# utiasSTARS/GraphIK

Hardware: AMD Instinct MI355X
Metric: IK solves/sec (batched random goals) (higher is better)
Workload: dtype f64

## Files before the change

graphik_amd/csrc/gik_rtr.hip.h:

```cpp
#pragma once

#include <hip/hip_runtime.h>

#include <type_traits>

#include "gik_wave.hip.h"

namespace gik {

#define UNI(cond) (__builtin_amdgcn_ballot_w64(cond) != 0ull)

__device__ inline bool plain_in_exec(double mv, double mp, double dHd, double e, double T, double beta, double rr,
                                     double t2hi, int j, int jmax_v) {
  unsigned long long ok, saved;
  asm volatile("s_mov_b64 %1, exec\n\t"
               "v_cmpx_lt_f64_e64 %0, %2, %3\n\t"
               "v_cmpx_gt_f64_e64 %0, %4, 0\n\t"
               "v_cmpx_gt_i32_e64 %0, %11, %10\n\t"
               "v_cmpx_lt_f64_e64 %0, %5, %6\n\t"
               "v_cmpx_ge_f64_e64 %0, %7, %8\n\t"
               "v_cmpx_nle_f64_e64 %0, %9, %12\n\t"
               "s_mov_b64 exec, %1"
               : "=&s"(ok), "=&s"(saved)
               : "s"(mv), "v"(mp), "s"(dHd), "v"(e), "v"(T), "v"(beta), "s"(1e-3), "v"(rr), "s"(j), "v"(jmax_v),
                 "v"(t2hi));
  return ok != 0ull;
}

struct RtrOut {
  double f, gradnorm;
  int iterations, inner_total, stop, n_accept;
  int inner_executed;
  double Delta;
  int paused;
};

struct RtrResume {
  double Delta;
  int kiter, inner_total, inner_exec, n_accept;
  int resumed;
  int resumes;
};

template <typename Ctx>
__device__ inline double grad_norm_and_rho(Ctx &cx, double g, double (&rho0)[Ctx::NC]) {
  if constexpr (Ctx::NC == 3) {
    double v[4] = {g * g, g * cx.Q[0], g * cx.Q[1], g * cx.Q[2]};
    cx.template sum_n<4>(v);
#pragma unroll
    for (int m = 0; m < 3; ++m) rho0[m] = v[m + 1];
    return sqrt(v[0]);
  }
  double v[Ctx::NC + 1];
  v[0] = g * g;
#pragma unroll
  for (int m = 0; m < Ctx::NC; ++m) v[m + 1] = g * cx.pk2[m];
  cx.template sum_n<Ctx::NC + 1>(v);
#pragma unroll
  for (int m = 0; m < Ctx::NC; ++m) rho0[m] = v[m + 1];
  return sqrt(v[0]);
}

__device__ inline double boundary_tau(double e_Pd2, double d_Pd, double Delta2, double e_Pe) {
  const double e_Pd = 0.5 * e_Pd2;
  return (sqrt(fma(e_Pd, e_Pd, d_Pd * (Delta2 - e_Pe))) - e_Pd) / d_Pd;
}

struct MigCtl {
  int *credits;
  int *simd_run;
  int sid;
  const unsigned int *fresh;
  const int *y_avail;
  const unsigned int *y_tail;
  int B;
  unsigned int y_cap;
  const unsigned int *done;
  int waves;
  int slice_cycles;
};
enum { PAUSE_NONE = 0, PAUSE_DONATE = 1, PAUSE_YIELD = 2 };

template <typename Ctx>
__device__ inline bool mig_poll(const Ctx &cx, const MigCtl &m) {
  int go = 0;
  if (cx.lead()) {
    if (__hip_atomic_load(m.credits, __ATOMIC_RELAXED, __HIP_MEMORY_SCOPE_AGENT) > 0 &&
        __hip_atomic_load(&m.simd_run[m.sid], __ATOMIC_RELAXED, __HIP_MEMORY_SCOPE_AGENT) >= 2) {
      if (__hip_atomic_fetch_add(m.credits, -1, __ATOMIC_RELAXED, __HIP_MEMORY_SCOPE_AGENT) >= 1)
        go = 1;
      else
        __hip_atomic_fetch_add(m.credits, 1, __ATOMIC_RELAXED, __HIP_MEMORY_SCOPE_AGENT);
    }
  }
  return __builtin_amdgcn_readfirstlane(go) != 0;
}

template <typename Ctx>
__device__ inline bool mig_anyone_waiting(const Ctx &cx, const MigCtl &m) {
  int w = 0;
  if (cx.lead()) {
    const unsigned int yt = __hip_atomic_load(m.y_tail, __ATOMIC_RELAXED, __HIP_MEMORY_SCOPE_AGENT);
    const unsigned int dn = __hip_atomic_load(m.done, __ATOMIC_RELAXED, __HIP_MEMORY_SCOPE_AGENT);
    w = yt + (unsigned)m.waves + 64u < m.y_cap && (unsigned)m.B > dn + (unsigned)m.waves;
  }
  return __builtin_amdgcn_readfirstlane(w) != 0;
}

template <typename Ctx, typename = void>
struct split_ehess : std::false_type {};
template <typename Ctx>
struct split_ehess<Ctx, std::enable_if_t<Ctx::SPLIT_EHESS>> : std::true_type {};

template <int K, bool THETA_ONE, bool SLICE, typename Ctx, bool MIG = false>
__device__ inline void rtr_solve_one(Ctx &cx, const Params &p, const gik_trace &trace, int has_trace,
                                     int dbg, double *dbg_buf, int b, double &x, RtrOut &out,
                                     const RtrResume &rs, int slice_its, const MigCtl *mig = nullptr) {
  static_assert(!MIG || SLICE, "tail spreading needs the resume / pause hooks");
  constexpr bool SPLIT = split_ehess<Ctx>::value && !MIG;
  constexpr bool EXEC_TEST = SPLIT && THETA_ONE;
  const double Delta_bar = 10.0 + K;
  const bool lead = cx.lead();
    double Delta = (SLICE && rs.resumed) ? rs.Delta : Delta_bar / 8.0;
    double fx = cx.cost(x);
    double g = cx.commit();
    cx.proj_setup(p.planar_proj_exact);
    double rho0[Ctx::NC];
    double norm_grad = grad_norm_and_rho(cx, g, rho0);
    int kiter = SLICE ? rs.kiter : 0, inner_total = SLICE ? rs.inner_total : 0,
        inner_exec = SLICE ? rs.inner_exec : 0, n_accept = SLICE ? rs.n_accept : 0, stop = 1;
    int slice_count = 0;
    long long slice_t0 = MIG ? (long long)__builtin_readcyclecounter() : 0;
    int paused = PAUSE_NONE;
    constexpr bool RETRACE = (K == 3) && Ctx::HAS_CK;
    const bool retrace_on = RETRACE && !(dbg & 16);
    bool prev_rejected = false, ck_set = false, ck_neg = false;
    int ck_j = 0;
    double ck_T = 0.0, ck_e_Pe = 0.0, ck_e_Pd2 = 0.0, ck_d_Pd = 0.0;
    double last_Delta2 = 0.0, last_e_Pe = 0.0;
    double eta = 0.0, Heta = 0.0;
    int stop_tCG = TCG_MAX_INNER_ITER, j = 0;
    const bool prof = (dbg & 8) && b == 0 && dbg_buf;
    long long prof_tcg = 0;
    const long long prof_t0 = prof ? (long long)__builtin_readcyclecounter() : 0;
    bool bad = UNI(!(fx == fx) || !(norm_grad == norm_grad));
    if (dbg & 2) bad = true;

    while (!bad) {
      if constexpr (Ctx::AGE_PRIORITY) {
        if (kiter == 32) __builtin_amdgcn_s_setprio(1);
        else if (kiter == 128) __builtin_amdgcn_s_setprio(2);
        else if (kiter == 512) __builtin_amdgcn_s_setprio(3);
        if constexpr (SLICE) {
          if (rs.resumed && slice_count == 0) {
            if (kiter > 512) __builtin_amdgcn_s_setprio(3);
            else if (kiter > 128) __builtin_amdgcn_s_setprio(2);
            else if (kiter > 32) __builtin_amdgcn_s_setprio(1);
          }
        }
      }
      const double Delta2 = Delta * Delta;
      bool reuse = false;
      if constexpr (RETRACE) {
        if (retrace_on && prev_rejected) {
          if (Delta2 == last_Delta2) {
            reuse = true;
          } else if (ck_set && Delta2 == ck_T) {
            const double tau = boundary_tau(ck_e_Pd2, ck_d_Pd, Delta2, ck_e_Pe);
            eta = fma(tau, cx.ck_get(2), cx.ck_get(0));
            Heta = fma(tau, cx.ck_get(3), cx.ck_get(1));
            stop_tCG = ck_neg ? TCG_NEGATIVE_CURVATURE : TCG_EXCEEDED_TR;
            j = ck_j;
            ck_set = false;
            reuse = true;
          } else if (stop_tCG != TCG_NEGATIVE_CURVATURE && stop_tCG != TCG_EXCEEDED_TR &&
                     last_e_Pe < Delta2) {
            reuse = true;
          }
        }
      }
      last_Delta2 = Delta2;
      const long long prof_t1 = prof ? (long long)__builtin_readcyclecounter() : 0;
      int executed = 0;
      if (reuse) {
      } else if constexpr (K == 3) {
        double eta_l = 0.0, Heta_l = 0.0;
        stop_tCG = TCG_MAX_INNER_ITER;
        int extra = 0;
        double r = g;
        const double r0_r0 = norm_grad * norm_grad;
        const double nr0_theta = (THETA_ONE || p.theta == 1.0) ? norm_grad : pow(norm_grad, p.theta);
        const double target = norm_grad * fmin(nr0_theta, p.kappa);
        const double target2 = target * target;
        const double target2_hi = target2 * (1.0 + 1e-9), target2_lo = target2 * (1.0 - 1e-9);
        const double Tq = 0.0625 * Delta2;
        double T_cur = RETRACE ? Tq : Delta2;
        ck_set = !RETRACE;
        double w = fma(rho0[2], cx.Q[2], fma(rho0[1], cx.Q[1], fma(rho0[0], cx.Q[0], -g)));
        double delta = w;
        double e_Pd2 = 0.0, d_Pd = r0_r0;
        double model_prev = __builtin_inf();
        double ea = 0.0, ha = 0.0, pa = 0.0;
        double eb = 0.0, hb = 0.0, pb = 0.0;
        double e_Pe_end = 0.0;
        __builtin_amdgcn_s_waitcnt(0);
        [[maybe_unused]] int maxinner_m1 = p.maxinner - 1;
        if constexpr (EXEC_TEST) asm volatile("" : "+v"(maxinner_m1));
        auto step = [&](const double ec, const double hc, const double pc, double &en, double &hn,
                        double &pn) __attribute__((always_inline)) -> bool {
          double H;
          if constexpr (SPLIT) H = cx.ehess_end();
          else H = cx.ehess(delta);
          double v[8] = {cx.Q[0] * H, cx.Q[1] * H, cx.Q[2] * H,      delta * H,
                         w * H,       H * H,       ec * fma(0.5, hc, g), r * r};
          double Hd_Hd;
          if constexpr (SPLIT) {
            const double wd = wave_sum8_distributed(v);
#pragma unroll
            for (int q = 0; q < 8; ++q)
              if (q != 5) v[q] = readlane_f64(wd, wave_sum8_lane(q));
            Hd_Hd = readlane_f64(fma(-v[2], v[2], fma(-v[1], v[1], fma(-v[0], v[0], wd))), wave_sum8_lane(5));
          } else {
            cx.template sum_n<8>(v);
            Hd_Hd = fma(-v[2], v[2], fma(-v[1], v[1], fma(-v[0], v[0], v[5])));
          }
          const double Hdelta = fma(-cx.Q[2], v[2], fma(-cx.Q[1], v[1], fma(-cx.Q[0], v[0], H)));
          const double d_Hd = v[3];
          const double model_value = v[6];
          const double r_r = v[7];
          const double rho = frcp1(d_Hd);
          const double alpha = r_r * rho;
#ifdef GIK_TCGDUMP
          if ((dbg & 4) && b == 0 && dbg_buf && kiter == 0) {
            const int slot = j < 256 ? j : 256 + (j >> 5);
            const double dq = cx.sum1(delta * cx.Q[0]), rq = cx.sum1(r * cx.Q[0]);
            if (slot < 1024 && lead) {
              double *q = dbg_buf + (size_t)slot * 8;
              q[0] = r_r; q[1] = d_Hd; q[2] = alpha; q[3] = model_value; q[4] = v[4]; q[5] = Hd_Hd;
              q[6] = dq; q[7] = rq;
            }
          }
#endif
          const double e_Pe_new = fma(alpha, fma(alpha, d_Pd, e_Pd2), pc);
          const double beta_p = fma(fma(alpha, Hd_Hd, -(v[4] + v[4])), rho, 1.0);
          double new_r_r = beta_p * r_r;
          bool leave;
          if constexpr (EXEC_TEST) {
            leave = !plain_in_exec(model_value, model_prev, d_Hd, e_Pe_new, T_cur, beta_p, new_r_r, target2_hi, j,
                                   maxinner_m1);
          } else {
            const bool rr_plain = SPLIT ? !(new_r_r <= target2_hi) : !((j >= p.mininner) & (new_r_r <= target2_hi));
            const bool plain = (model_value < model_prev) & (d_Hd > 0.0) & (e_Pe_new < T_cur) & (beta_p >= 1e-3) &
                               rr_plain & (j + 1 < p.maxinner);
            leave = UNI(!plain);
          }
          double beta = beta_p;
          double rr_test = new_r_r;
          if (__builtin_expect(leave, 0)) {
            if (!(d_Hd == d_Hd) || !(new_r_r == new_r_r) || !(model_value == model_value)) {
              bad = true;
              return true;
            }
            if (model_value >= model_prev) {
              eta_l = en;
              Heta_l = hn;
              e_Pe_end = pc;
              stop_tCG = TCG_MODEL_INCREASED;
              extra = 1;
              j = j - 1;
              return true;
            }
            if constexpr (RETRACE) {
              if (!ck_set && (d_Hd <= 0.0 || e_Pe_new >= Tq)) {
                cx.ck_put(0, ec);
                cx.ck_put(1, hc);
                cx.ck_put(2, delta);
                cx.ck_put(3, Hdelta);
                ck_e_Pe = pc;
                ck_e_Pd2 = e_Pd2;
                ck_d_Pd = d_Pd;
                ck_j = j;
                ck_neg = d_Hd <= 0.0;
                ck_T = Tq;
                ck_set = true;
                T_cur = Delta2;
              }
            }
            if (d_Hd <= 0.0 || e_Pe_new >= Delta2) {
              const double tau = boundary_tau(e_Pd2, d_Pd, Delta2, pc);
              eta_l = fma(tau, delta, ec);
              Heta_l = fma(tau, Hdelta, hc);
              e_Pe_end = pc;
              stop_tCG = (d_Hd <= 0.0) ? TCG_NEGATIVE_CURVATURE : TCG_EXCEEDED_TR;
              return true;
            }
            double alpha_c = alpha;
            asm volatile("" : "+v"(alpha_c));
            if (beta_p < 1e-3) {
              const double new_r = fma(alpha_c, Hdelta, r);
              new_r_r = cx.sum1(new_r * new_r);
              beta = new_r_r / r_r;
              rr_test = new_r_r;
            } else if (j >= p.mininner && new_r_r >= target2_lo && new_r_r <= target2_hi) {
              const double new_r = fma(alpha_c, Hdelta, r);
              rr_test = cx.sum1(new_r * new_r);
            }
            if (j >= p.mininner && rr_test <= target2) {
              e_Pe_end = e_Pe_new;
              const double new_eta = fma(alpha_c, delta, ec);
              const double new_Heta = fma(alpha_c, Hdelta, hc);
              const double model_new = cx.sum1(new_eta * fma(0.5, new_Heta, g));
              if (model_new >= model_value) {
                eta_l = ec;
                Heta_l = hc;
                stop_tCG = TCG_MODEL_INCREASED;
              } else {
                eta_l = new_eta;
                Heta_l = new_Heta;
                stop_tCG = (p.kappa < nr0_theta) ? TCG_REACHED_TARGET_LINEAR
                                                 : TCG_REACHED_TARGET_SUPERLINEAR;
              }
              return true;
            }
            if (j + 1 >= p.maxinner) {
              e_Pe_end = e_Pe_new;
              const double new_eta = fma(alpha_c, delta, ec);
              const double new_Heta = fma(alpha_c, Hdelta, hc);
              const double model_last = cx.sum1(new_eta * fma(0.5, new_Heta, g));
              if (model_last >= model_value) {
                eta_l = ec;
                Heta_l = hc;
                stop_tCG = TCG_MODEL_INCREASED;
              } else {
                eta_l = new_eta;
                Heta_l = new_Heta;
              }
              j = p.maxinner;
              return true;
            }
          }
          ++j;
          pn = e_Pe_new;
          model_prev = model_value;
          if constexpr (SPLIT) {
            en = fma(alpha, delta, ec);
            w = fma(-alpha, Hdelta, w);
            delta = fma(beta, delta, w);
            cx.ehess_begin(delta);
            __builtin_amdgcn_sched_barrier(0);
            hn = fma(alpha, Hdelta, hc);
            r = fma(alpha, Hdelta, r);
          } else {
            en = fma(alpha, delta, ec);
            hn = fma(alpha, Hdelta, hc);
            r = fma(alpha, Hdelta, r);
            w = fma(-alpha, Hdelta, w);
            delta = fma(beta, delta, w);
          }
          e_Pd2 = beta * fma(alpha + alpha, d_Pd, e_Pd2);
          d_Pd = fma(beta * beta, d_Pd, new_r_r);
          return false;
        };
        j = 0;
        if constexpr (SPLIT) {
          if (p.maxinner > 0) cx.ehess_begin(delta);
        }
        if (p.maxinner > 0)
          for (;;) {
            if (step(ea, ha, pa, eb, hb, pb)) break;
            if (step(eb, hb, pb, ea, ha, pa)) break;
          }
        const double e_Pe = e_Pe_end;
        last_e_Pe = e_Pe;
        eta = eta_l;
        Heta = Heta_l;
        executed = (j >= p.maxinner ? p.maxinner : j + 1) + extra;
      } else {
        eta = 0.0;
        Heta = 0.0;
        stop_tCG = TCG_MAX_INNER_ITER;
        double r = g;
        double e_Pe = 0.0;
        double r_r = cx.sum1(r * r);
        const double norm_r0 = sqrt(r_r);
        const double nr0_theta = (THETA_ONE || p.theta == 1.0) ? norm_r0 : pow(norm_r0, p.theta);
        const double target = norm_r0 * fmin(nr0_theta, p.kappa);
        const double target2 = target * target;
        double z_r = r_r, d_Pd = r_r;
        double inv_z_r = frcp(z_r);
        double delta = -r;
        double e_Pd = 0.0, model_value = 0.0;
        double rho_pk[Ctx::NC], s_pk[Ctx::NC], hd_pk[Ctx::NC];
#pragma unroll
        for (int m = 0; m < Ctx::NC; ++m) {
          rho_pk[m] = rho0[m];
          s_pk[m] = -rho0[m];
        }
        for (j = 0; j < p.maxinner; ++j) {
          double d_Hd;
          const double Hdelta = cx.hess_proj_dot(delta, s_pk, d_Hd, hd_pk);
          if (UNI(!(d_Hd == d_Hd))) { bad = true; break; }
          const double alpha = z_r * frcp(d_Hd);
          const double e_Pe_new = e_Pe + 2.0 * alpha * e_Pd + alpha * alpha * d_Pd;
          if (UNI(d_Hd <= 0.0 || e_Pe_new >= Delta * Delta)) {
            const double tau =
                (-e_Pd + sqrt(e_Pd * e_Pd + d_Pd * (Delta * Delta - e_Pe))) / d_Pd;
            eta = eta + tau * delta;
            Heta = Heta + tau * Hdelta;
            stop_tCG = (d_Hd <= 0.0) ? TCG_NEGATIVE_CURVATURE : TCG_EXCEEDED_TR;
            break;
          }
          if ((dbg & 4) && b == 0 && lead && dbg_buf && kiter < 64 && j < 128) {
            double *q = dbg_buf + ((size_t)kiter * 128 + j) * 4;
            q[0] = r_r; q[1] = d_Hd; q[2] = alpha; q[3] = model_value;
          }
          e_Pe = e_Pe_new;
          const double new_eta = eta + alpha * delta;
          const double new_Heta = Heta + alpha * Hdelta;
          const double new_r = r + alpha * Hdelta;
          double m[3] = {new_eta * g, new_eta * new_Heta, new_r * new_r};
          cx.template sum_n<3>(m);
          const double new_model_value = m[0] + 0.5 * m[1];
          if (UNI(new_model_value >= model_value)) {
            stop_tCG = TCG_MODEL_INCREASED;
            break;
          }
          eta = new_eta;
          Heta = new_Heta;
          model_value = new_model_value;
          r = new_r;
          r_r = m[2];
          if (UNI(j >= p.mininner && r_r <= target2)) {
            stop_tCG = (p.kappa < nr0_theta) ? TCG_REACHED_TARGET_LINEAR
                                             : TCG_REACHED_TARGET_SUPERLINEAR;
            break;
          }
          z_r = r_r;
          const double beta = z_r * inv_z_r;
          inv_z_r = frcp(z_r);
          delta = -r + beta * delta;
          if constexpr (K == 2) {
#pragma unroll
            for (int m = 0; m < Ctx::NC; ++m) {
              rho_pk[m] = fma(alpha, hd_pk[m], rho_pk[m]);
              s_pk[m] = fma(beta, s_pk[m], -rho_pk[m]);
            }
          }
          e_Pd = beta * (e_Pd + alpha * d_Pd);
          d_Pd = z_r + beta * beta * d_Pd;
        }
        executed = j >= p.maxinner ? p.maxinner : j + 1;
      }
      if (prof) prof_tcg += (long long)__builtin_readcyclecounter() - prof_t1;
      if (bad) break;
      if (j >= p.maxinner) j = p.maxinner - 1;
      inner_total += j + 1;
      inner_exec += executed;

      if (has_trace && kiter < trace.cap && lead) {
        const size_t q = (size_t)b * trace.cap + kiter;
        trace.d_Delta[q] = Delta;
        trace.d_numit[q] = j;
        trace.d_stop[q] = stop_tCG;
        trace.d_f_before[q] = fx;
      }
      const double x_prop = x + eta;
      const double fx_prop = cx.cost(x_prop);
      double rhonum = fx - fx_prop;
      double gd[2] = {g * eta, eta * Heta};
      cx.template sum_n<2>(gd);
      double rhoden = -gd[0] - 0.5 * gd[1];
      const double rho_reg =
          fmax(1.0, fabs(fx)) * 2.220446049250313e-16 * p.rho_regularization;
      rhonum += rho_reg;
      rhoden += rho_reg;
      const bool model_decreased = rhoden >= 0.0;
      const double rho = rhonum / rhoden;
      if (rho < 0.25 || !model_decreased || !(rho == rho)) {
        Delta = Delta / 4.0;
      } else if (rho > 0.75 &&
                 (stop_tCG == TCG_NEGATIVE_CURVATURE || stop_tCG == TCG_EXCEEDED_TR)) {
        Delta = fmin(2.0 * Delta, Delta_bar);
      }
      int accept = 0;
      prev_rejected = true;
      if (UNI(model_decreased && rho > p.rho_prime)) {
        accept = 1;
        prev_rejected = false;
        ++n_accept;
        x = x_prop;
        fx = fx_prop;
        g = cx.commit();
        cx.proj_setup(p.planar_proj_exact);
        norm_grad = grad_norm_and_rho(cx, g, rho0);
      }
      if (has_trace && kiter < trace.cap && lead) {
        const size_t q = (size_t)b * trace.cap + kiter;
        trace.d_gradnorm_after[q] = norm_grad;
        trace.d_accept[q] = accept;
      }
      kiter = kiter + 1;
      if (kiter >= p.maxiter) { stop = 1; break; }
      if (UNI(norm_grad < p.mingradnorm)) { stop = 0; break; }
      if (UNI(!(norm_grad == norm_grad) || !(fx == fx))) { bad = true; break; }
      if constexpr (MIG) {
        ++slice_count;
        if ((kiter & 3) == 0 && mig_poll(cx, *mig)) { paused = PAUSE_DONATE; break; }
        if (slice_its > 0 && slice_count >= slice_its &&
            (long long)__builtin_readcyclecounter() - slice_t0 > (long long)mig->slice_cycles) {
          if (mig_anyone_waiting(cx, *mig)) { paused = PAUSE_YIELD; break; }
          slice_count = 0;
          slice_t0 = (long long)__builtin_readcyclecounter();
        }
      } else if constexpr (SLICE) {
        if (slice_its > 0 && ++slice_count >= slice_its) { paused = PAUSE_YIELD; break; }
      }
    }
    if (bad) stop = 2;
    if constexpr (Ctx::AGE_PRIORITY) __builtin_amdgcn_s_setprio(0);
    if (prof && lead) {
      dbg_buf[0] = (double)prof_tcg;
      dbg_buf[1] = (double)inner_total;
      dbg_buf[2] = (double)((long long)__builtin_readcyclecounter() - prof_t0);
      dbg_buf[3] = (double)inner_exec;
    }

    out.f = fx;
    out.gradnorm = norm_grad;
    out.iterations = kiter;
    out.inner_total = inner_total;
    out.inner_executed = inner_exec;
    out.stop = stop;
    out.n_accept = n_accept;
    out.Delta = Delta;
    out.paused = paused;
}

}
```

graphik_amd/csrc/gik_wave_strict.hip.h:

```cpp
#pragma once

#include "gik_wave.hip.h"

namespace gik {

template <int MAXDEG>
struct WaveCtxStrict : WaveCtx<3, MAXDEG, false, true> {
  using Base = WaveCtx<3, MAXDEG, false, true>;
  using SlotRec = typename Base::SlotRec;
  static constexpr int K = 3;
  static constexpr int RS = Base::RS;
  static constexpr int NSH = Base::NSL;
  static constexpr bool HAS_CK = Base::HAS_CK;
  static constexpr bool AGE_PRIORITY = Base::AGE_PRIORITY;

  int natoff[NSH];
  double ysn[NSH][3];
  double cc[NSH];

  __device__ inline void init(int lane_, int N, double *tiles, const double *tgt, uint32_t *meta) {
    Base::init(lane_, N, tiles, tgt, meta);
#pragma unroll
    for (int k = 0; k < NSH; ++k) {
      natoff[k] = meta_j(this->sh_meta[k * WAVE + this->lane]) * RS;
      cc[k] = ysn[k][0] = ysn[k][1] = ysn[k][2] = 0.0;
    }
  }

  __device__ inline SlotRec record(int k) const { return this->sh_rec[k * WAVE + this->lane]; }

  __device__ inline double triple_sum(const double (&p)[3]) const {
    const double a0 = wave_shl<1>(p[0]), b0 = wave_shl<1>(a0);
    const double a1 = wave_shl<1>(p[1]), c1 = wave_shr<1>(p[1]);
    const double c2 = wave_shr<1>(p[2]), d2 = wave_shr<1>(c2);
    const double t0 = (p[0] + a0) + b0;
    const double t1 = (c1 + p[1]) + a1;
    const double t2 = (d2 + c2) + p[2];
    return bit_select(this->comp == 0, t0, bit_select(this->comp == 1, t1, t2));
  }

  __device__ inline double cost(double Yv) {
    this->put1(Yv);
    const Row<3> own = this->read_row(this->nat_off);
    double f = 0.0;
#pragma unroll
    for (int k = 0; k < NSH; ++k) {
      const Row<3> r = this->read_row(natoff[k]);
      const SlotRec rc = record(k);
      const double y0 = own.v[0] - r.v[0], y1 = own.v[1] - r.v[1], y2 = own.v[2] - r.v[2];
      const double d = fma(y2, y2, fma(y1, y1, y0 * y0));
      const double cl = fmin(fmax(rc.tg - d, (double)rc.lo), (double)rc.hi);
      f = fma(cl, cl, f);
    }
    return 0.5 * wave_sum(this->active ? f : 0.0);
  }

  __device__ inline double commit() {
    const Row<3> own = this->read_row(this->nat_off);
    double gp[3] = {0.0, 0.0, 0.0};
#pragma unroll
    for (int k = 0; k < NSH; ++k) {
      const Row<3> r = this->read_row(natoff[k]);
      const SlotRec rc = record(k);
      const double y0 = own.v[0] - r.v[0], y1 = own.v[1] - r.v[1], y2 = own.v[2] - r.v[2];
      const double d = fma(y2, y2, fma(y1, y1, y0 * y0));
      const double cl = fmin(fmax(rc.tg - d, (double)rc.lo), (double)rc.hi);
      const bool act = (rc.lo * rc.hi < 0.0f) || (cl != 0.0);
      const double c = -cl;
      ysn[k][0] = act ? y0 + y0 : 0.0;
      ysn[k][1] = act ? y1 + y1 : 0.0;
      ysn[k][2] = act ? y2 + y2 : 0.0;
      cc[k] = c + c;
      gp[0] = fma(c, y0, gp[0]);
      gp[1] = fma(c, y1, gp[1]);
      gp[2] = fma(c, y2, gp[2]);
    }
    return 2.0 * triple_sum(gp);
  }

  static constexpr bool SPLIT_EHESS = true;
  Row<3> wn_, rw_[NSH];
  __device__ inline void ehess_begin(double W) {
    this->put1(W);
    wn_ = this->read_row(this->nat_off);
#pragma unroll
    for (int k = 0; k < NSH; ++k) rw_[k] = this->read_row(natoff[k]);
  }
  __device__ inline double ehess_end() {
    double p[3] = {0.0, 0.0, 0.0};
#pragma unroll
    for (int k = 0; k < NSH; ++k) {
      const double u0 = wn_.v[0] - rw_[k].v[0], u1 = wn_.v[1] - rw_[k].v[1], u2 = wn_.v[2] - rw_[k].v[2];
      const double s = fma(ysn[k][2], u2, fma(ysn[k][1], u1, ysn[k][0] * u0));
      p[0] = fma(s, ysn[k][0], fma(cc[k], u0, p[0]));
      p[1] = fma(s, ysn[k][1], fma(cc[k], u1, p[1]));
      p[2] = fma(s, ysn[k][2], fma(cc[k], u2, p[2]));
    }
    return triple_sum(p);
  }
  __device__ inline double ehess(double W) {
    ehess_begin(W);
    return ehess_end();
  }

  __device__ inline double hess_proj_dot(double delta, const double (&s_dpk)[3], double &d_Hd, double (&hd_pk)[3]) {
    return this->proj_dot(ehess(delta), delta, s_dpk, d_Hd, hd_pk);
  }
};

}
```

Measured before the change: 44720.

## Split tCG inner loop into hot test/update path with cold exit handling

For strict wave contexts with three slots and the exec-test path, the truncated-CG inner loop is restructured into a hot loop that only runs a fused exec-mask test and the state update. All rare exit checks (NaN, model increase, boundary, residual target, checkpointing) move into a cold path that runs only when the fast test fails. A slotwise Hessian end variant adds scheduling barriers to order the loads. This aims to shrink the per-iteration instruction count and branch divergence, but it duplicates logic and the exit semantics must match the original step exactly.

```diff
diff --git a/graphik_amd/csrc/gik_rtr.hip.h b/graphik_amd/csrc/gik_rtr.hip.h
--- a/graphik_amd/csrc/gik_rtr.hip.h
+++ b/graphik_amd/csrc/gik_rtr.hip.h
@@ -112,6 +112,11 @@
 template <typename Ctx>
 struct split_ehess<Ctx, std::enable_if_t<Ctx::SPLIT_EHESS>> : std::true_type {};
 
+template <typename Ctx, bool EXEC_TEST, typename = void>
+struct lone_loop : std::false_type {};
+template <typename Ctx>
+struct lone_loop<Ctx, true, std::enable_if_t<Ctx::NSH == 3>> : std::true_type {};
+
 template <int K, bool THETA_ONE, bool SLICE, typename Ctx, bool MIG = false>
 __device__ inline void rtr_solve_one(Ctx &cx, const Params &p, const gik_trace &trace, int has_trace,
                                      int dbg, double *dbg_buf, int b, double &x, RtrOut &out,
@@ -119,6 +124,7 @@
   static_assert(!MIG || SLICE, "tail spreading needs the resume / pause hooks");
   constexpr bool SPLIT = split_ehess<Ctx>::value && !MIG;
   constexpr bool EXEC_TEST = SPLIT && THETA_ONE;
+  constexpr bool LONE_LOOP = lone_loop<Ctx, EXEC_TEST>::value;
   const double Delta_bar = 10.0 + K;
   const bool lead = cx.lead();
     double Delta = (SLICE && rs.resumed) ? rs.Delta : Delta_bar / 8.0;
@@ -365,7 +371,152 @@
         if constexpr (SPLIT) {
           if (p.maxinner > 0) cx.ehess_begin(delta);
         }
-        if (p.maxinner > 0)
+        if constexpr (LONE_LOOP) {
+          (void)step;
+          double Hdelta, d_Hd, model_value, r_r, alpha, e_Pe_new, beta_p, new_r_r, beta, rr_test;
+          auto step_test = [&](const double ec, const double hc, const double pc) __attribute__((always_inline)) -> bool {
+            const double H = cx.ehess_end_slotwise();
+            double v[8] = {cx.Q[0] * H, cx.Q[1] * H, cx.Q[2] * H,      delta * H,
+                           w * H,       H * H,       ec * fma(0.5, hc, g), r * r};
+            const double wd = wave_sum8_distributed(v);
+#pragma unroll
+            for (int q = 0; q < 8; ++q)
+              if (q != 5) v[q] = readlane_f64(wd, wave_sum8_lane(q));
+            const double Hd_Hd = readlane_f64(fma(-v[2], v[2], fma(-v[1], v[1], fma(-v[0], v[0], wd))), wave_sum8_lane(5));
+            Hdelta = fma(-cx.Q[2], v[2], fma(-cx.Q[1], v[1], fma(-cx.Q[0], v[0], H)));
+            d_Hd = v[3];
+            model_value = v[6];
+            r_r = v[7];
+            const double rho = frcp1(d_Hd);
+            alpha = r_r * rho;
+            e_Pe_new = fma(alpha, fma(alpha, d_Pd, e_Pd2), pc);
+            beta_p = fma(fma(alpha, Hd_Hd, -(v[4] + v[4])), rho, 1.0);
+            new_r_r = beta_p * r_r;
+            beta = beta_p;
+            rr_test = new_r_r;
+            return !plain_in_exec(model_value, model_prev, d_Hd, e_Pe_new, T_cur, beta_p, new_r_r, target2_hi, j, maxinner_m1);
+          };
+          auto step_cold = [&](const double ec, const double hc, const double pc, const double en,
+                               const double hn) __attribute__((always_inline)) -> bool {
+            if (!(d_Hd == d_Hd) || !(new_r_r == new_r_r) || !(model_value == model_value)) {
+              bad = true;
+              return true;
+            }
+            if (model_value >= model_prev) {
+              eta_l = en;
+              Heta_l = hn;
+              e_Pe_end = pc;
+              stop_tCG = TCG_MODEL_INCREASED;
+              extra = 1;
+              j = j - 1;
+              return true;
+            }
+            if constexpr (RETRACE) {
+              if (!ck_set && (d_Hd <= 0.0 || e_Pe_new >= Tq)) {
+                cx.ck_put(0, ec);
+                cx.ck_put(1, hc);
+                cx.ck_put(2, delta);
+                cx.ck_put(3, Hdelta);
+                ck_e_Pe = pc;
+                ck_e_Pd2 = e_Pd2;
+                ck_d_Pd = d_Pd;
+                ck_j = j;
+                ck_neg = d_Hd <= 0.0;
+                ck_T = Tq;
+                ck_set = true;
+                T_cur = Delta2;
+              }
+            }
+            if (d_Hd <= 0.0 || e_Pe_new >= Delta2) {
+              const double tau = boundary_tau(e_Pd2, d_Pd, Delta2, pc);
+              eta_l = fma(tau, delta, ec);
+              Heta_l = fma(tau, Hdelta, hc);
+              e_Pe_end = pc;
+              stop_tCG = (d_Hd <= 0.0) ? TCG_NEGATIVE_CURVATURE : TCG_EXCEEDED_TR;
+              return true;
+            }
+            double alpha_c = alpha;
+            asm volatile("" : "+v"(alpha_c));
+            if (beta_p < 1e-3) {
+              const double new_r = fma(alpha_c, Hdelta, r);
+              new_r_r = cx.sum1(new_r * new_r);
+              beta = new_r_r / r_r;
+              rr_test = new_r_r;
+            } else if (j >= p.mininner && new_r_r >= target2_lo && new_r_r <= target2_hi) {
+              const double new_r = fma(alpha_c, Hdelta, r);
+              rr_test = cx.sum1(new_r * new_r);
+            }
+            if (j >= p.mininner && rr_test <= target2) {
+              e_Pe_end = e_Pe_new;
+              const double new_eta = fma(alpha_c, delta, ec);
+              const double new_Heta = fma(alpha_c, Hdelta, hc);
+              const double model_new = cx.sum1(new_eta * fma(0.5, new_Heta, g));
+              if (model_new >= model_value) {
+                eta_l = ec;
+                Heta_l = hc;
+                stop_tCG = TCG_MODEL_INCREASED;
+              } else {
+                eta_l = new_eta;
+                Heta_l = new_Heta;
+                stop_tCG = (p.kappa < nr0_theta) ? TCG_REACHED_TARGET_LINEAR
+                                                 : TCG_REACHED_TARGET_SUPERLINEAR;
+              }
+              return true;
+            }
+            if (j + 1 >= p.maxinner) {
+              e_Pe_end = e_Pe_new;
+              const double new_eta = fma(alpha_c, delta, ec);
+              const double new_Heta = fma(alpha_c, Hdelta, hc);
+              const double model_last = cx.sum1(new_eta * fma(0.5, new_Heta, g));
+              if (model_last >= model_value) {
+                eta_l = ec;
+                Heta_l = hc;
+                stop_tCG = TCG_MODEL_INCREASED;
+              } else {
+                eta_l = new_eta;
+                Heta_l = new_Heta;
+              }
+              j = p.maxinner;
+              return true;
+            }
+            return false;
+          };
+          auto step_update = [&](const double ec, const double hc, double &en, double &hn, double &pn)
+                                 __attribute__((always_inline)) {
+            ++j;
+            pn = e_Pe_new;
+            model_prev = model_value;
+            en = fma(alpha, delta, ec);
+            w = fma(-alpha, Hdelta, w);
+            delta = fma(beta, delta, w);
+            cx.ehess_begin(delta);
+            __builtin_amdgcn_sched_barrier(0);
+            hn = fma(alpha, Hdelta, hc);
+            r = fma(alpha, Hdelta, r);
+            e_Pd2 = beta * fma(alpha + alpha, d_Pd, e_Pd2);
+            d_Pd = fma(beta * beta, d_Pd, new_r_r);
+          };
+          auto swap_sets = [&]() __attribute__((always_inline)) {
+            double t;
+            t = ea, ea = eb, eb = t;
+            t = ha, ha = hb, hb = t;
+            t = pa, pa = pb, pb = t;
+          };
+          if (p.maxinner > 0)
+            for (;;) {
+              bool second;
+              for (;;) {
+                if (__builtin_expect(step_test(ea, ha, pa), 0)) { second = false; break; }
+                step_update(ea, ha, eb, hb, pb);
+                if (__builtin_expect(step_test(eb, hb, pb), 0)) { second = true; break; }
+                step_update(eb, hb, ea, ha, pa);
+              }
+              if (second) swap_sets();
+              if (step_cold(ea, ha, pa, eb, hb)) break;
+              step_update(ea, ha, eb, hb, pb);
+              swap_sets();
+            }
+        } else if (p.maxinner > 0)
           for (;;) {
             if (step(ea, ha, pa, eb, hb, pb)) break;
             if (step(eb, hb, pb, ea, ha, pa)) break;
diff --git a/graphik_amd/csrc/gik_wave_strict.hip.h b/graphik_amd/csrc/gik_wave_strict.hip.h
--- a/graphik_amd/csrc/gik_wave_strict.hip.h
+++ b/graphik_amd/csrc/gik_wave_strict.hip.h
@@ -98,6 +98,20 @@
     }
     return triple_sum(p);
   }
+  __device__ inline double ehess_end_slotwise() {
+    double p[3] = {0.0, 0.0, 0.0};
+#pragma unroll
+    for (int k = 0; k < NSH; ++k) {
+      const double u2 = wn_.v[2] - rw_[k].v[2];
+      __builtin_amdgcn_sched_barrier(0);
+      const double u0 = wn_.v[0] - rw_[k].v[0], u1 = wn_.v[1] - rw_[k].v[1];
+      const double s = fma(ysn[k][2], u2, fma(ysn[k][1], u1, ysn[k][0] * u0));
+      p[0] = fma(s, ysn[k][0], fma(cc[k], u0, p[0]));
+      p[1] = fma(s, ysn[k][1], fma(cc[k], u1, p[1]));
+      p[2] = fma(s, ysn[k][2], fma(cc[k], u2, p[2]));
+    }
+    return triple_sum(p);
+  }
   __device__ inline double ehess(double W) {
     ehess_begin(W);
     return ehess_end();
```

Measured after the change: 46450, median of 6. 3.9% higher.
